# Sota0726/weather-Unet

Hardware: AMD Instinct MI355X
Metric: images/sec 256x256 cUNet fwd+bwd (higher is better)
Workload: dtype bf16; 1 GPU; cUNet 256x256 bf16 B=32/GPU, training step: fwd + bwd (dgrad+wgrad) + grad all-reduce + fused Adam; dropout p=0.3 on; random-init weights, 5-class one-hot, loss mean|G(x,c)-x|; global_batch=32, parallelism=dp1

## Files before the change

include/wu_kernels.h:

```cpp
#ifndef WU_KERNELS_H
#define WU_KERNELS_H

#include <stddef.h>
#include <stdint.h>

#ifdef __cplusplus
extern "C" {
#endif

#define WU_F32 0
#define WU_BF16 1

#define WU_ACT_NONE 0
#define WU_ACT_RELU 1
#define WU_ACT_LEAKY 2

const char* wu_last_error(void);
int wu_version(void);
int wu_cu_count(void);
int wu_set_option(int key, int value);
int wu_set_debug_buffer(void* p);
int wu_event_create(void** event_out);
int wu_event_destroy(void* event);
int wu_stream_order_after(void* waiter_stream, void* producer_stream, void* event);

int wu_stream_create_cu_mask(const unsigned* mask, int words, void** stream_out);
int wu_stream_destroy(void* stream);

int wu_pack_conv3x3(const float* w_oihw, void* w_fwd, void* w_dgrad, int Cout, int Cin,
                    const float* inv_sigma, int dtype, void* stream);
int wu_pack_conv3x3_multi(int n, const float* const* w_oihw, void* const* w_fwd, void* const* w_dgrad,
                          const int* Cout, const int* Cin, int dtype, void* stream);

size_t wu_spectral_norm_scratch_floats(int rows, int cols);
int wu_spectral_norm_fwd(const float* w, int rows, int cols, float* u, float* v, int power_iter, float eps,
                         float* sigma_out, float* w_eff, float* scratch, void* stream);
int wu_spectral_norm_bwd(const float* g, const float* w, const float* u, const float* v, const float* sigma,
                         float* dw, int rows, int cols, float* scratch, void* stream);
int wu_spectral_norm_fwd_multi(int n, const float* const* w, const int* rows, const int* cols, float* const* u, float* const* v,
                               int power_iter, float eps, float* const* sigma_out, float* const* w_eff, float* const* scratch,
                               float* const* u_save, float* const* v_save, void* stream);
int wu_spectral_norm_bwd_multi(int n, const float* const* g, const float* const* w, const float* const* u, const float* const* v,
                               const float* const* sigma, float* const* dw, const int* rows, const int* cols, float* const* scratch,
                               void* stream);

int wu_conv3x3_fwd(const void* x, int ldx, const void* w_packed, const float* bias, void* y, int ldy,
                   int N, int H, int W, int Cin, int Cout, int stride, int act,
                   const void* mask, int ldmask, int mask_act,
                   const void* egate, int ldegate, int egate_act, int dtype, void* stream);

int wu_conv3x3_gate_bits_supported(int H, int W, int ldx, int ldy, int Cin, int Cout, int dtype);
size_t wu_gate_bits_bytes(int N, int H, int W, int C);
int wu_conv3x3_fwd_bits(const void* x, int ldx, const void* w_packed, const float* bias, void* y, int ldy,
                        void* gate_bits_out, const void* egate_bits, int N, int H, int W, int Cin, int Cout,
                        int act, int dtype, void* stream);

int wu_conv3x3_relu_pool_fwd(const void* x, int ldx, const void* w_packed, const float* bias, void* y, int ldy,
                             void* pool, int ldpool, int N, int H, int W, int Cin, int Cout, int dtype, void* stream);
int wu_conv3x3_relu_pool_bits_fwd(const void* x, int ldx, const void* w_packed, const float* bias, void* y, int ldy,
                                  void* pool, int ldpool, void* gate_bits_out, void* sel_bits_out,
                                  int N, int H, int W, int Cin, int Cout, int dtype, void* stream);
int wu_conv3x3_small_supported(int N, int H, int W, int ldx, int ldy, int ldegate, int Cin, int Cout);
int wu_conv3x3_small_fwd(const void* x, int ldx, const void* w_chunked, const float* bias, void* y, int ldy,
                         const void* egate, int ldegate, int egate_act, int N, int H, int W, int Cin, int Cout, int act, void* stream);

int wu_conv3x3_relu_head_supported(int H, int W, int ldx, int ldy, int Cin, int Cout, int dtype);
int wu_conv3x3_relu_head_fwd(const void* x, int ldx, const void* w_packed, const float* bias, void* y, int ldy,
                             const float* head_w, const float* head_bias, float* out_nchw,
                             int N, int H, int W, int Cin, int Cout, int dtype, void* stream);
int wu_maxpool2_bwd_bits(const unsigned* gate_bits, const unsigned* sel_bits, const void* dy, int lddy, const void* dskip, int lddskip,
                         void* dx, int lddx, int N, int H, int W, int C, int dtype, void* stream);

size_t wu_conv3x3_wgrad_workspace(int N, int H, int W, int Cin, int Cout, int stride, int dtype);
int wu_conv3x3_wgrad(const void* x, int ldx, const void* dy, int lddy, const void* y, int ldy_, int act,
                     float* dw_oihw, float* dbias, void* workspace, size_t workspace_bytes,
                     int N, int H, int W, int Cin, int Cout, int stride, int accumulate,
                     int dtype, void* stream);

size_t wu_conv3x3_s2_dgrad_workspace(int N, int H, int W, int Cout, int dtype);
int wu_conv3x3_s2_dgrad(const void* dy, int lddy, const void* y, int ldy_, int act, const void* w_dgrad,
                        void* dx, int lddx, void* workspace, size_t workspace_bytes,
                        const void* egate, int ldegate, int egate_act,
                        int N, int H, int W, int Cin, int Cout, int dtype, void* stream);

int wu_act_gate(const void* g, int ldg, const void* y, int ldy, void* out, int ldo,
                int N, int H, int W, int C, int act, int dtype, void* stream);

int wu_conv3x3_c3_fwd(const float* x_nchw, const float* w_oihw, const float* bias, const float* inv_sigma,
                      void* y, int ldy, int out_nchw, int N, int H, int W, int Cout, int stride, int act,
                      int dtype, void* stream);
int wu_conv3x3_c3_gate_bits_supported(int N, int H, int W, int Cout, int stride, const float* bias, int dtype);
int wu_conv3x3_c3_fwd_bits(const float* x_nchw, const float* w_oihw, const float* bias, const float* inv_sigma,
                           void* y, int ldy, void* gate_bits_out, int N, int H, int W, int Cout, int stride, int dtype, void* stream);
int wu_conv3x3_c3_wgrad(const float* x_nchw, const void* dy, int lddy, int dy_nchw, const void* y, int ldy_,
                        int act, float* dw_oihw, float* dbias, void* workspace, size_t workspace_bytes,
                        int N, int H, int W, int Cout, int stride, int accumulate, int dtype, void* stream);
size_t wu_thin_workspace_bytes(void);
int wu_conv3x3_c3_dgrad(const void* dy, int lddy, int dy_nchw, const void* y, int ldy_, int act,
                        const float* w_oihw, const float* inv_sigma, float* dx_nchw, int N, int H, int W,
                        int Cout, int stride, int accumulate, int dtype, void* stream);

int wu_conv1x1_tanh_fwd(const void* x, int ldx, const float* w, const float* bias, float* out_nchw,
                        int N, int H, int W, int Cin, int dtype, void* stream);
int wu_conv1x1_tanh_bwd(const float* dout_nchw, const float* out_nchw, const void* x, int ldx, const float* w,
                        void* dx, int lddx, float* dw, float* dbias, void* workspace, size_t workspace_bytes,
                        int N, int H, int W, int Cin, int accumulate, int x_gate_act, int dtype, void* stream);

int wu_maxpool2_fwd(const void* x, int ldx, void* y, int ldy, int N, int H, int W, int C, int dtype, void* stream);
int wu_maxpool2_bwd(const void* x, int ldx, const void* dy, int lddy, const void* dskip, int lddskip,
                    void* dx, int lddx, int N, int H, int W, int C, int gate_act, int dtype, void* stream);

int wu_adain_style_fwd(const float* y, const float* w, const float* b, float eps, float* y_std, float* y_mean, float* y4,
                       int N, int C, int nc, void* stream);
int wu_adain_style_bwd(const float* d_std, const float* d_mean, const float* y, const float* y4, const float* y_std,
                       const float* y_mean, float* dw, float* db, int N, int C, int nc, int accumulate, void* stream);

int wu_adain_style_fwd_multi(int levels, const float* y, const float* const* w, const float* const* b, const float* eps,
                             float* const* y_std, float* const* y_mean, float* const* y4, int N, const int* C, int nc, void* stream);
int wu_adain_style_bwd_multi(int levels, const float* const* d_std, const float* const* d_mean, const float* y, const float* const* y4,
                             const float* const* y_std, const float* const* y_mean, float* const* dw, float* const* db,
                             int N, const int* C, int nc, int accumulate, void* stream);

#define WU_MAX_SPLITS 16
int wu_adain_stats(const void* x, int ldx, float* stats, float* scratch, int N, int H, int W, int C,
                   float eps, int dtype, void* stream);
int wu_adain_stats_as_batch(const void* x, int ldx, float* stats, float* scratch, int N, int H, int W, int C,
                            float eps, int split_batch, int dtype, void* stream);

int wu_adain_upcat_fwd(const void* x, int ldx, const float* stats, const float* y_std, const float* y_mean,
                       void* y, int ldy, int N, int H, int W, int C, float p_drop, uint64_t seed,
                       const uint64_t* seed_dev, uint8_t* mask_bits, int mask_is_input, int dtype, void* stream);
int wu_adain_upcat_sweep_fwd(const void* x, int ldx, int Bx, const float* stats, const float* y_std, const float* y_mean,
                             const void* skip, int ldskip, int Bs, int Cs, void* y, int ldy, int N, int H, int W, int C,
                             float p_drop, uint64_t seed, const uint64_t* seed_dev, int dtype, void* stream);
int wu_adain_upcat_bwd(const void* dy, int lddy, const void* x, int ldx, const float* stats, const float* y_std,
// ... 333 lines not shown
```

weather-unet_amd/csrc/conv3x3_mfma_v2.hip:

```cpp
#include <type_traits>

#include "wu_common.h"
#include "conv_internal.h"

#ifndef WU_CONV_STORE_AUX
#define WU_CONV_STORE_AUX 0
#endif

namespace {

struct K {
    static constexpr int TH = 16, TW = 32, P = TH * TW;
    static constexpr int HALO_W = TW + 2, HALO_H = TH + 2, HALO_PIX = HALO_W * HALO_H;
    static constexpr int H_PIECES = 40, H_BYTES = H_PIECES * 1024;
    static constexpr int W_REAL = 9 * 64 * 64 / 1024;
    static constexpr int W_PIECES = 40, W_BYTES = W_PIECES * 1024;
    static constexpr int BUF = H_BYTES + W_BYTES;
};
template <int NW_> struct KW {
    static constexpr int NW = NW_;
    static constexpr int RPW = K::TH / NW;
    static constexpr int NH = K::H_PIECES / NW;
    static constexpr int NWT = K::W_PIECES / NW;
    static constexpr int NP = NH + NWT;
    static constexpr int NST = K::P * 8 / (NW * 64);
};

struct V2Args {
    const bf16_t* x; const bf16_t* w; const float* bias; bf16_t* y; const bf16_t* egate;
    bf16_t* pool;
    unsigned* gbits;
    unsigned* sbits;
    const unsigned* egbits;
    int ldx, ldy, ldegate, egate_act, ldpool;
    int N, H, W, Cin, Cout, act;
    int tiles_x, tiles_y, cout_tiles, ntiles, prio_mode, strided;
    int w_resident;
    const float* head_w; const float* head_b; float* head_out;
    unsigned long long* dbg;
};

typedef float f32x2_t __attribute__((ext_vector_type(2)));
typedef short s16x2_t __attribute__((ext_vector_type(2)));
typedef unsigned short u16x2_t __attribute__((ext_vector_type(2)));
__device__ __forceinline__ uint32_t relu_bf16x2(uint32_t d) {
    const s16x2_t v = __builtin_elementwise_max(__builtin_bit_cast(s16x2_t, d), s16x2_t{0, 0});
    return __builtin_bit_cast(uint32_t, v);
}
__device__ __forceinline__ uint32_t relu_gate_bf16x2(uint32_t g, uint32_t y) {
    const u16x2_t nz = __builtin_elementwise_min(__builtin_bit_cast(u16x2_t, y), u16x2_t{1, 1});
    const u16x2_t m = u16x2_t{0, 0} - nz;
    const s16x2_t sg = __builtin_bit_cast(s16x2_t, y) >> s16x2_t{15, 15};
    return g & __builtin_bit_cast(uint32_t, m) & ~__builtin_bit_cast(uint32_t, sg);
}
__device__ __forceinline__ uint32_t max_u16x2(uint32_t a, uint32_t b) {
    const u16x2_t m = __builtin_elementwise_max(__builtin_bit_cast(u16x2_t, a), __builtin_bit_cast(u16x2_t, b));
    return __builtin_bit_cast(uint32_t, m);
}
__device__ __forceinline__ uint32_t nonzero_byte(const uint4& v) {
    uint32_t t0, t1, t2, t3;
    const uint32_t one = 0x00010001u;
    asm("v_pk_min_u16 %0, %1, %2" : "=&v"(t0) : "v"(v.x), "v"(one));
    asm("v_pk_min_u16 %0, %1, %2" : "=&v"(t1) : "v"(v.y), "v"(one));
    asm("v_pk_min_u16 %0, %1, %2" : "=&v"(t2) : "v"(v.z), "v"(one));
    asm("v_pk_min_u16 %0, %1, %2" : "=&v"(t3) : "v"(v.w), "v"(one));
    const uint32_t xx = ((t3 << 6) | t2 << 4) | ((t1 << 2) | t0);
    return (xx | (xx >> 15)) & 0xffu;
}
__device__ __forceinline__ uint32_t gate_mask2(int bits, int b) {
    const uint32_t lo = (uint32_t)((bits << (31 - b)) >> 31), hi = (uint32_t)((bits << (30 - b)) >> 31);
    return (lo & 0xffffu) | (hi << 16);
}
__device__ __forceinline__ float fast_tanh(float s) {
    const float e = __builtin_amdgcn_exp2f(s * 2.885390081777927f);
    return 1.f - 2.f * __builtin_amdgcn_rcpf(e + 1.f);
}
__device__ __forceinline__ void dma_wait_all() { asm volatile("s_waitcnt vmcnt(0)" ::: "memory"); }
__device__ __forceinline__ void mma(f32x16_t& acc, const uint4& a, const uint4& b) {
    acc = __builtin_amdgcn_mfma_f32_32x32x16_bf16(__builtin_bit_cast(bf16x8_t, a), __builtin_bit_cast(bf16x8_t, b), acc, 0, 0, 0);
}
__device__ __forceinline__ void mma16(f32x4_t& acc, const uint4& a, const uint4& b) {
    acc = __builtin_amdgcn_mfma_f32_16x16x32_bf16(__builtin_bit_cast(bf16x8_t, a), __builtin_bit_cast(bf16x8_t, b), acc, 0, 0, 0);
}
template <bool M16_, int RPW_> struct AccT { using type = f32x16_t[RPW_][2]; };
template <int RPW_> struct AccT<true, RPW_> { using type = f32x4_t[RPW_][2][4]; };

template <int NW, int GATED>
__global__ __launch_bounds__(NW * 64) void conv3x3_mfma_v2_kernel(const V2Args a) {
    using Q = KW<NW>;
// ... 272 lines not shown
                    load_step(1, af[1], bf[1]);
                    __builtin_amdgcn_sched_barrier(0);
                    mma_step(2);
                    __builtin_amdgcn_sched_barrier(0);
                }
#pragma unroll
                for (int step = 0; step < 18; ++step) {
                    if (step + 2 < 18) load_step(step + 2, af[(step + 2) % 3], bf[(step + 2) % 3]);
                    if (more && 2 * step < Q::NP) {
                        if (need_w || 2 * step < Q::NH) issue_piece(2 * step, c1, nxt);
                        if (2 * step + 1 < Q::NP && (need_w || 2 * step + 1 < Q::NH)) issue_piece(2 * step + 1, c1, nxt);
                    }
                    static_assert(2 * 5 >= Q::NP || NW != 8, "deferred stores must follow the last DMA piece");
                    if (FIRST && ov_pending && (GATED != 5 || has_y) && step >= 5 && step < 5 + Q::NST) store_ov(step - 5);
                    if (GATED == 3 && FIRST && ovb_pending && step >= 5 + Q::NST && step < 5 + Q::NST + Q::RPW) store_ovb(step - 5 - Q::NST);
                    if (GATED == 5 && FIRST && ovh_pending && step >= 5 + Q::NST && 2 * (step - 5 - Q::NST) < 3 * Q::RPW) {
                        store_ovh(2 * (step - 5 - Q::NST));
                        if (2 * (step - 5 - Q::NST) + 1 < 3 * Q::RPW) store_ovh(2 * (step - 5 - Q::NST) + 1);
                    }
                    __builtin_amdgcn_sched_barrier(0);
                    if (LAST || step < 18 - CARRY) mma_step(step % 3);
                    __builtin_amdgcn_sched_barrier(0);
                }
            } else {
                constexpr int NF = 12, NM = 32;
                auto load_frag = [&](int tap, int f, uint4 (&xf)[Q::RPW][2], uint4 (&wf)[4]) __attribute__((always_inline)) {
                    const int kh = tap / 3, kw = tap % 3;
                    if (f == 0 || f >= 9) {
                        const int cb = f == 0 ? 0 : f - 8;
                        wf[cb] = *(const uint4*)(lds + b16_lane + (tap * 64 + 16 * cb) * 64);
                    } else {
                        const int mi = (f - 1) >> 1, ph = (f - 1) & 1;
                        xf[mi][ph] = *(const uint4*)(lds + a16_lane[kw] + ((mi + kh) * K::HALO_W + 16 * ph) * 64);
                    }
                };
                auto mma_m = [&](int m, int slot) __attribute__((always_inline)) {
                    const int cb = m >> 3, mi = (m & 7) >> 1, ph = m & 1;
                    mma16(acc[mi][ph][cb], wr[slot][cb], xr[slot][mi][ph]);
                };
                const unsigned kill = more ? 0u : kWuOOB;
                if constexpr (FIRST) {
#pragma unroll
                    for (int f = 0; f < NF; ++f) load_frag(0, f, xr[0], wr[0]);
                } else {
#pragma unroll
                    for (int m = 0; m < NM; ++m) {
                        mma_m(m, 2);
                        if (m < NF) load_frag(0, m, xr[0], wr[0]);
                        __builtin_amdgcn_sched_barrier(0);
                    }
                }
#pragma unroll
                for (int tap = 0; tap < 9; ++tap) {
                    const int cur = tap % 3, nx = (tap + 1) % 3;
#pragma unroll
                    for (int m = 0; m < NM; ++m) {
                        if (LAST || tap < 9 - CARRY) mma_m(m, cur);
                        if (tap + 1 < 9 && m < NF) load_frag(tap + 1, m, xr[nx], wr[nx]);
                        if ((m == 15 || m == NM - 1) && 4 * tap < Q::NP) {
                            const int j0 = 4 * tap + (m == 15 ? 0 : 2);
                            if (j0 < Q::NP) issue_piece(j0, c1, nxt, kill);
                            if (j0 + 1 < Q::NP) issue_piece(j0 + 1, c1, nxt, kill);
                        }
                        static_assert(4 * 5 >= Q::NP || NW != 4, "deferred stores must follow the last DMA piece");
                        if (FIRST && (m == 15 || m == NM - 1) && ov_pending && tap >= 5) {
                            const int k0 = 4 * (tap - 5) + (m == 15 ? 0 : 2);
                            if (k0 + 1 < Q::NST) { store_ov(k0); store_ov(k0 + 1); }
                        }
                        if (GATED == 3 && FIRST && m == NM - 1 && ovb_pending && tap == 8) {
#pragma unroll
                            for (int mi = 0; mi < Q::RPW; ++mi) store_ovb(mi);
                        }
                        __builtin_amdgcn_sched_barrier(0);
                    }
                }
            }
            buf = nxt;
            if (FIRST && ov_pending) { stores_in_flight = ov_interior; bits_in_flight = ovb_pending; ov_pending = false; ovb_pending = false; ovh_pending = false; }
            if (FIRST) WU_STAMP(t_comp); else WU_STAMP(t_comp_rest);
        };
        do_chunk(0, std::true_type{}, std::false_type{});
        for (int c = 1; c + 1 < nchunks; ++c) do_chunk(c, std::false_type{}, std::false_type{});
        do_chunk(nchunks - 1, std::false_type{}, std::true_type{});
        if constexpr (M16) __syncthreads();

        const int n = cur.n;
        const int oh0 = cur.ty * K::TH, ow0 = cur.tx * K::TW, co0 = cur.ct * 64;
        WU_STAMP(t_epi_b1);
        const size_t img_pix = (size_t)n * a.H * a.W;
        auto epi_store = [&](auto act_tag, auto eg_tag, auto pool_tag) __attribute__((always_inline)) {
            constexpr int ACT = decltype(act_tag)::value, EG = decltype(eg_tag)::value;
            constexpr bool POOL = decltype(pool_tag)::value;
            constexpr int SCR_PITCH = 144;
            char* const scr = smem + (buf ^ 1) * K::BUF + wave * (Q::RPW * 32 * SCR_PITCH);
            if constexpr (M16) {
                static_assert(NW * Q::RPW * 32 * SCR_PITCH <= K::BUF, "transpose scratch must fit the free LDS buffer");
#pragma unroll
                for (int mi = 0; mi < Q::RPW; ++mi)
#pragma unroll
                    for (int ph = 0; ph < 2; ++ph)
#pragma unroll
                        for (int cb = 0; cb < 4; ++cb) {
                            const float4 bv = (GATED == 1 || GATED == 2) ? make_float4(0.f, 0.f, 0.f, 0.f) : b16[cb];
                            f32x2_t v0 = f32x2_t{acc[mi][ph][cb][0], acc[mi][ph][cb][1]} + f32x2_t{bv.x, bv.y};
                            f32x2_t v1 = f32x2_t{acc[mi][ph][cb][2], acc[mi][ph][cb][3]} + f32x2_t{bv.z, bv.w};
                            if (ACT == WU_ACT_LEAKY) {
                                const f32x2_t s0_ = v0 * 0.2f, s1_ = v1 * 0.2f;
                                v0 = f32x2_t{fmaxf(v0.x, s0_.x), fmaxf(v0.y, s0_.y)};
                                v1 = f32x2_t{fmaxf(v1.x, s1_.x), fmaxf(v1.y, s1_.y)};
                            }
                            uint2 o = make_uint2(pack_bf16x2(v0.x, v0.y), pack_bf16x2(v1.x, v1.y));
                            if (ACT == WU_ACT_RELU) { o.x = relu_bf16x2(o.x); o.y = relu_bf16x2(o.y); }
                            *(uint2*)(scr + (mi * 32 + 16 * ph + l15) * SCR_PITCH + (16 * cb + 4 * q16) * 2) = o;
                        }
            }
            unsigned gb[Q::RPW], sb[Q::RPW];
#pragma unroll
            for (int i = 0; i < Q::RPW; ++i) gb[i] = sb[i] = 0u;
            f32x16_t hacc[Q::RPW];
            if constexpr (GATED == 5) {
#pragma unroll
                for (int mi = 0; mi < Q::RPW; ++mi)
#pragma unroll
                    for (int i = 0; i < 16; ++i) hacc[mi][i] = 0.f;
            }
#pragma unroll
            for (int mp = 0; mp < Q::RPW / 2; ++mp) {
                const int ohe = oh0 + Q::RPW * wave + 2 * mp, ow = ow0 + l31;
#pragma unroll
                for (int ni = 0; ni < 2; ++ni)
#pragma unroll
                    for (int g = 0; g < 4; g += 2) {
                        uint4 vr[2];
#pragma unroll
                        for (int r = 0; r < 2; ++r) {
                            const int mi = 2 * mp + r;
                            uint4 v;
                            if constexpr (M16) {
                                v = *(const uint4*)(scr + (mi * 32 + l31) * SCR_PITCH + (32 * ni + 8 * g + 8 * lh) * 2);
                            } else {
                            uint32_t o[2][2];
#pragma unroll
                            for (int h = 0; h < 2; ++h) {
                                const float4 bv = (GATED == 1 || GATED == 2) ? make_float4(0.f, 0.f, 0.f, 0.f) : bvq[ni][g + h];
                                const int r0 = 4 * (g + h);
                                f32x2_t v0 = f32x2_t{acc[mi][ni][r0 + 0], acc[mi][ni][r0 + 1]} + f32x2_t{bv.x, bv.y};
                                f32x2_t v1 = f32x2_t{acc[mi][ni][r0 + 2], acc[mi][ni][r0 + 3]} + f32x2_t{bv.z, bv.w};
                                if (ACT == WU_ACT_LEAKY) {
                                    const f32x2_t s0_ = v0 * 0.2f, s1_ = v1 * 0.2f;
                                    v0 = f32x2_t{fmaxf(v0.x, s0_.x), fmaxf(v0.y, s0_.y)};
                                    v1 = f32x2_t{fmaxf(v1.x, s1_.x), fmaxf(v1.y, s1_.y)};
                                }
                                o[h][0] = pack_bf16x2(v0.x, v0.y);
                                o[h][1] = pack_bf16x2(v1.x, v1.y);
                                if (ACT == WU_ACT_RELU) { o[h][0] = relu_bf16x2(o[h][0]); o[h][1] = relu_bf16x2(o[h][1]); }
                            }
                            const auto s0 = __builtin_amdgcn_permlane32_swap(o[0][0], o[1][0], false, false);
                            const auto s1 = __builtin_amdgcn_permlane32_swap(o[0][1], o[1][1], false, false);
                            v = make_uint4(s0[0], s1[0], s0[1], s1[1]);
                            }
                            if (GATED == 2) {
                                const int by = (int)(egb[mi] >> (8 * (2 * ni + (g >> 1))));
                                v.x &= gate_mask2(by, 0);
                                v.y &= gate_mask2(by, 2);
                                v.z &= gate_mask2(by, 4);
                                v.w &= gate_mask2(by, 6);
                            } else if (EG != WU_ACT_NONE) {
                                const uint4 yv = egv[mi][ni][g >> 1];
                                if (EG == WU_ACT_RELU) {
                                    v.x = relu_gate_bf16x2(v.x, yv.x); v.y = relu_gate_bf16x2(v.y, yv.y);
                                    v.z = relu_gate_bf16x2(v.z, yv.z); v.w = relu_gate_bf16x2(v.w, yv.w);
                                } else {
                                    v = gate16<bf16_t>(v, yv, WU_ACT_LEAKY);
                                }
                            }
                            ov[((mp * 2 + ni) * 2 + (g >> 1)) * 2 + r] = v;
                            vr[r] = v;
                            if constexpr (GATED == 5) mma(hacc[mi], hA[2 * ni + (g >> 1)], v);
                            if ((GATED == 3 || GATED == 4) && ACT == WU_ACT_RELU)
                                gb[2 * mp + r] |= nonzero_byte(v) << (8 * (2 * ni + (g >> 1)));
                        }
                        if (POOL) {
                            uint4 m = make_uint4(max_u16x2(vr[0].x, vr[1].x), max_u16x2(vr[0].y, vr[1].y), max_u16x2(vr[0].z, vr[1].z), max_u16x2(vr[0].w, vr[1].w));
                            m.x = max_u16x2(m.x, (uint32_t)__builtin_amdgcn_mov_dpp((int)m.x, 0xB1, 0xF, 0xF, true));
                            m.y = max_u16x2(m.y, (uint32_t)__builtin_amdgcn_mov_dpp((int)m.y, 0xB1, 0xF, 0xF, true));
                            m.z = max_u16x2(m.z, (uint32_t)__builtin_amdgcn_mov_dpp((int)m.z, 0xB1, 0xF, 0xF, true));
                            m.w = max_u16x2(m.w, (uint32_t)__builtin_amdgcn_mov_dpp((int)m.w, 0xB1, 0xF, 0xF, true));
                            if ((l31 & 1) == 0 && ohe + 1 < a.H && ow + 1 < a.W) {
                                const int Hp = a.H >> 1, Wp = a.W >> 1;
                                *(uint4*)(a.pool + (((size_t)n * Hp + (ohe >> 1)) * Wp + (ow >> 1)) * a.ldpool + co0 + 8 * lh + 32 * ni + 8 * g) = m;
                            }
                            if constexpr (GATED == 4) {
                                const uint4 x0 = make_uint4(vr[0].x ^ m.x, vr[0].y ^ m.y, vr[0].z ^ m.z, vr[0].w ^ m.w);
                                const uint4 x1 = make_uint4(vr[1].x ^ m.x, vr[1].y ^ m.y, vr[1].z ^ m.z, vr[1].w ^ m.w);
                                const uint32_t eq0 = ~nonzero_byte(x0) & 0xffu, eq1 = ~nonzero_byte(x1) & 0xffu;
                                const uint32_t nb = (uint32_t)__builtin_amdgcn_mov_dpp((int)(eq0 | (eq1 << 8)), 0xB1, 0xF, 0xF, true);
                                const uint32_t oddm = (l31 & 1) ? 0xffu : 0u;
                                const uint32_t nb0 = nb & 0xffu, nb1 = (nb >> 8) & 0xffu;
                                const uint32_t s0 = eq0 & ~(nb0 & oddm);
                                const uint32_t s1 = eq1 & ~eq0 & ~nb0 & ~(nb1 & oddm);
                                sb[2 * mp] |= s0 << (8 * (2 * ni + (g >> 1)));
                                sb[2 * mp + 1] |= s1 << (8 * (2 * ni + (g >> 1)));
                            }
                        }
                    }
            }
            if constexpr (GATED == 4) {
#pragma unroll
                for (int mi = 0; mi < Q::RPW; ++mi) {
                    const int oh = oh0 + Q::RPW * wave + mi, ow = ow0 + l31;
                    if (oh < a.H && ow < a.W) {
                        const size_t wi = (((size_t)n * a.H + oh) * a.W + ow) * (2 * a.cout_tiles) + 2 * cur.ct + lh;
                        a.gbits[wi] = gb[mi];
                        a.sbits[wi] = sb[mi];
                    }
                }
            }
            if constexpr (GATED == 5) {
#pragma unroll
                for (int mi = 0; mi < Q::RPW; ++mi)
#pragma unroll
                    for (int c = 0; c < 3; ++c) ovh[mi][c] = fast_tanh((hacc[mi][c] + (hacc[mi][4 + c] + hacc[mi][8 + c])) + hbias[c]);
                ovh_off = (unsigned)(((size_t)n * 3 * a.H + oh0 + Q::RPW * wave) * a.W + ow0 + l31);
                ovh_pending = true;
            }
            if (GATED == 3 && ACT == WU_ACT_RELU) {
#pragma unroll
                for (int mi = 0; mi < Q::RPW; ++mi) ovb[mi] = gb[mi];
                ovb_off = (unsigned)((((size_t)n * a.H + oh0 + Q::RPW * wave) * a.W + ow0 + l31) * (2 * a.cout_tiles) + 2 * cur.ct + lh);
                ovb_pending = true;
            }
        };
        using A0 = std::integral_constant<int, WU_ACT_NONE>;
        using A1 = std::integral_constant<int, WU_ACT_RELU>;
        using A2 = std::integral_constant<int, WU_ACT_LEAKY>;
        using NoPool = std::false_type;
        if constexpr (GATED == 5) {
            epi_store(A1{}, A0{}, NoPool{});
        } else if constexpr (GATED == 4) {
            epi_store(A1{}, A0{}, std::true_type{});
        } else if constexpr (GATED == 3) {
            epi_store(A1{}, A0{}, NoPool{});
        } else if constexpr (GATED == 2) {
            epi_store(A0{}, A0{}, NoPool{});
        } else if constexpr (GATED == 1) {
            if (a.egate_act == WU_ACT_RELU) epi_store(A0{}, A1{}, NoPool{});
            else epi_store(A0{}, A2{}, NoPool{});
        } else {
            if (a.act == WU_ACT_RELU) {
                if (a.pool) epi_store(A1{}, A0{}, std::true_type{});
                else epi_store(A1{}, A0{}, NoPool{});
            }
            else if (a.act == WU_ACT_LEAKY) epi_store(A2{}, A0{}, NoPool{});
            else epi_store(A0{}, A0{}, NoPool{});
        }
        {
            const int ohw = oh0 + Q::RPW * wave, ow = ow0 + l31;
            ov_img = has_y ? a.y + img_pix * a.ldy : a.y;
            ov_off = (unsigned)(((ohw * a.W + ow) * a.ldy + co0 + 8 * lh) * 2);
            unsigned rows = 0;
#pragma unroll
            for (int rr = 0; rr < Q::RPW; ++rr) rows |= (ohw + rr < a.H && ow < a.W) ? (1u << rr) : 0u;
            ov_ok = 0;
#pragma unroll
            for (int k = 0; k < Q::NST; ++k) ov_ok |= ((rows >> (2 * (k >> 3) + (k & 1))) & 1u) << k;
            ov_interior = oh0 + K::TH <= a.H && ow0 + K::TW <= a.W;
            ov_pending = true;
        }
        WU_STAMP(t_epi_s);
        cur = advance(cur);
    }
    if (ov_pending) {
        if (GATED != 5 || has_y) {
#pragma unroll
            for (int k = 0; k < Q::NST; ++k) store_ov(k);
        }
        if (GATED == 5 && ovh_pending) {
#pragma unroll
            for (int k = 0; k < 3 * Q::RPW; ++k) store_ovh(k);
        }
        if (GATED == 3 && ovb_pending) {
#pragma unroll
            for (int mi = 0; mi < Q::RPW; ++mi) store_ovb(mi);
        }
    }
    if (NW == 4) dma_wait_all();
    if (a.dbg && lane == 0) {
        unsigned long long* d = a.dbg + ((size_t)blockIdx.x * 8 + wave) * 8;
        d[0] = t_wait; d[1] = t_comp + t_comp_rest; d[2] = __builtin_readcyclecounter() - t_k0; d[3] = __builtin_amdgcn_s_memrealtime() - t_r0;
         d[4] = t_epi_b2; d[5] = t_epi_s; d[6] = (unsigned long long)((t_end - t_begin + t_step - 1) / t_step); d[7] = nchunks | (t_comp << 8);
    }
#undef WU_STAMP
}

}

bool conv_v2_eligible(int H, int W, int ldx, int ldy, int Cin, int Cout, int stride, int dtype, bool masked) {
    return dtype == WU_BF16 && stride == 1 && !masked && W > 16 && W <= 4096 && Cin % 32 == 0 && Cin >= 64 && Cout % 64 == 0 &&
           (size_t)9 * Cout * Cin * 2 < (1ull << 31) && ((size_t)H * W + W + 2) * (size_t)ldx * 2 < (1ull << 31) &&
           ((size_t)H * W + W + 2) * (size_t)ldy * 2 < (1ull << 31);
}

int conv_v2_launch(const void* x, int ldx, const void* w, const float* bias, void* y, int ldy,
                   const void* egate, int ldegate, int egate_act, int N, int H, int W, int Cin, int Cout, int act, hipStream_t s,
                   void* pool, int ldpool, void* gate_bits_out, const void* egate_bits, void* sel_bits_out,
                   const float* head_w, const float* head_b, float* head_out) {
    V2Args a;
    a.head_w = head_w; a.head_b = head_b; a.head_out = head_out;
    a.pool = (bf16_t*)pool; a.ldpool = ldpool;
    a.x = (const bf16_t*)x; a.w = (const bf16_t*)w; a.bias = bias; a.y = (bf16_t*)y; a.egate = (const bf16_t*)egate;
    a.ldx = ldx; a.ldy = ldy; a.ldegate = ldegate; a.egate_act = egate_act; a.N = N; a.H = H; a.W = W; a.Cin = Cin; a.Cout = Cout; a.act = act;
    a.tiles_x = cdiv(W, K::TW); a.tiles_y = cdiv(H, K::TH); a.cout_tiles = Cout / 64;
    a.dbg = (unsigned long long*)g_wu_dbg_ptr;
    a.prio_mode = g_wu_opt[WU_OPT_CONV_PRIO];
    a.strided = g_wu_opt[WU_OPT_CONV_STRIDED];
    a.w_resident = 0;
    const long long ntiles = (long long)N * a.tiles_x * a.tiles_y * a.cout_tiles;
    if (ntiles >= (1ll << 31)) return -1;
    a.ntiles = (int)ntiles;
    const int cus = wu_num_cus();
    const long long grid = (ntiles < cus || !g_wu_opt[WU_OPT_CONV_PERSISTENT]) ? ntiles : cus;
    static thread_local bool attr_set = false;
    if (!attr_set) {
#define WU_V2_ATTR(NW_, G_) (void)hipFuncSetAttribute((const void*)conv3x3_mfma_v2_kernel<NW_, G_>, hipFuncAttributeMaxDynamicSharedMemorySize, 160 * 1024)
        WU_V2_ATTR(8, 5); WU_V2_ATTR(8, 0); WU_V2_ATTR(4, 0); WU_V2_ATTR(8, 1); WU_V2_ATTR(4, 1); WU_V2_ATTR(8, 2); WU_V2_ATTR(4, 2); WU_V2_ATTR(8, 3); WU_V2_ATTR(4, 3); WU_V2_ATTR(8, 4); WU_V2_ATTR(4, 4);
#undef WU_V2_ATTR
        attr_set = true;
    }
    const int mode = g_wu_opt[WU_OPT_CONV_V2];
    int gated = egate_bits ? 2 : ((egate != nullptr && egate_act != WU_ACT_NONE) ? 1 : 0);
    if (gated != 1) a.egate = nullptr;
    a.egbits = (const unsigned*)egate_bits;
    a.gbits = (gated == 0 && act == WU_ACT_RELU && !pool) ? (unsigned*)gate_bits_out : nullptr;
    a.sbits = nullptr;
    if (a.gbits) gated = 3;
    if (gated == 0 && act == WU_ACT_RELU && pool && gate_bits_out && sel_bits_out) {
        a.gbits = (unsigned*)gate_bits_out; a.sbits = (unsigned*)sel_bits_out;
        gated = 4;
    }
    if (head_out) {
        if (gated != 0 || act != WU_ACT_RELU || pool || Cout != 64 || Cin >= 256) return -2;
        gated = 5;
    }
    const bool nw4 = gated != 5 && (mode == 2 || (mode == 1 && Cin >= 256));
    a.w_resident = (!nw4 && Cin == 64 && a.cout_tiles == 1 && g_wu_opt[WU_OPT_CONV_W_RESIDENT]) ? 1 : 0;
#define WU_V2_GO(NW_, G_) hipLaunchKernelGGL((conv3x3_mfma_v2_kernel<NW_, G_>), dim3((int)grid), dim3(NW_ * 64), 2 * K::BUF, s, a)
    if (nw4) { if (gated == 4) WU_V2_GO(4, 4); else if (gated == 3) WU_V2_GO(4, 3); else if (gated == 2) WU_V2_GO(4, 2); else if (gated == 1) WU_V2_GO(4, 1); else WU_V2_GO(4, 0); }
    else { if (gated == 5) WU_V2_GO(8, 5); else if (gated == 4) WU_V2_GO(8, 4); else if (gated == 3) WU_V2_GO(8, 3); else if (gated == 2) WU_V2_GO(8, 2); else if (gated == 1) WU_V2_GO(8, 1); else WU_V2_GO(8, 0); }
#undef WU_V2_GO
    return 0;
}
```

weather-unet_amd/wu/_lib.py:

```python
import ctypes
import os

from ctypes import c_char_p, c_double, c_float, c_int, c_size_t, c_uint64, c_void_p, POINTER

_PKG = os.path.dirname(os.path.dirname(os.path.abspath(__file__)))
LIB_PATH = os.path.join(_PKG, "lib", "libwu_kernels.so")

F32, BF16 = 0, 1
ACT_NONE, ACT_RELU, ACT_LEAKY = 0, 1, 2
OPT_CONV_V2, OPT_CONV_PERSISTENT, OPT_WGRAD_V2 = 0, 1, 2
FAM_CONV_FWD, FAM_WGRAD, FAM_CONV_DGRAD, FAM_CONV_S2, FAM_WGRAD_S2, FAM_CONV1X1 = 1, 2, 3, 4, 5, 6
FAM_GRID = 7
FAMILY_KERNEL = {1: "conv3x3_mfma_v2_kernel (forward + data-gradient convs; generic conv3x3_mfma_kernel for fp32 / narrow images)",
                 2: "conv3x3_wgrad_v2_kernel (generic conv3x3_wgrad_kernel for fp32 / narrow images)",
                 3: "conv3x3_mfma_kernel<T,1,true> (in-kernel gated dgrad; unused by the fused graph)",
                 4: "stride-2 3x3 conv forward + data gradient: conv1x1_pw3_kernel<.., CONV> (gathered rows); conv3x3_mfma_kernel<T,2,false> / tap-list classes for 64-cout and fp32",
                 5: "conv3x3_wgrad_kernel<T,2>",
                 6: "pointwise convs (estimator): conv1x1_pw3_kernel; conv1x1_mfma_kernel<T> for strided / small / fp32"}

P, I, F, U64, SZ = c_void_p, c_int, c_float, c_uint64, c_size_t

SIGNATURES = {
    "wu_last_error": (c_char_p, []),
    "wu_version": (I, []),
    "wu_cu_count": (I, []),
    "wu_set_option": (I, [I, I]),
    "wu_set_debug_buffer": (I, [P]),
    "wu_stream_create_cu_mask": (I, [P, I, P]),
    "wu_stream_destroy": (I, [P]),
    "wu_spectral_norm_scratch_floats": (SZ, [I, I]),
    "wu_spectral_norm_fwd": (I, [P, I, I, P, P, I, F, P, P, P, P]),
    "wu_spectral_norm_bwd": (I, [P, P, P, P, P, P, I, I, P, P]),
    "wu_event_create": (I, [P]),
    "wu_event_destroy": (I, [P]),
    "wu_stream_order_after": (I, [P, P, P]),
    "wu_spectral_norm_fwd_multi": (I, [I, P, P, P, P, P, I, F, P, P, P, P, P, P]),
    "wu_spectral_norm_bwd_multi": (I, [I, P, P, P, P, P, P, P, P, P, P]),
    "wu_pack_conv3x3": (I, [P, P, P, I, I, P, I, P]),
    "wu_pack_conv3x3_multi": (I, [I, P, P, P, P, P, I, P]),
    "wu_conv3x3_fwd": (I, [P, I, P, P, P, I, I, I, I, I, I, I, I, P, I, I, P, I, I, I, P]),
    "wu_conv3x3_gate_bits_supported": (I, [I, I, I, I, I, I, I]),
    "wu_gate_bits_bytes": (SZ, [I, I, I, I]),
    "wu_conv3x3_fwd_bits": (I, [P, I, P, P, P, I, P, P, I, I, I, I, I, I, I, P]),
    "wu_conv3x3_relu_pool_fwd": (I, [P, I, P, P, P, I, P, I, I, I, I, I, I, I, P]),
    "wu_conv3x3_relu_pool_bits_fwd": (I, [P, I, P, P, P, I, P, I, P, P, I, I, I, I, I, I, P]),
    "wu_conv3x3_small_supported": (I, [I, I, I, I, I, I, I, I]),
    "wu_conv3x3_small_fwd": (I, [P, I, P, P, P, I, P, I, I, I, I, I, I, I, I, P]),
    "wu_conv3x3_relu_head_supported": (I, [I, I, I, I, I, I, I]),
    "wu_conv3x3_relu_head_fwd": (I, [P, I, P, P, P, I, P, P, P, I, I, I, I, I, I, P]),
    "wu_maxpool2_bwd_bits": (I, [P, P, P, I, P, I, P, I, I, I, I, I, I, P]),
    "wu_conv3x3_wgrad_workspace": (SZ, [I, I, I, I, I, I, I]),
    "wu_conv3x3_wgrad": (I, [P, I, P, I, P, I, I, P, P, P, SZ, I, I, I, I, I, I, I, I, P]),
    "wu_conv3x3_s2_dgrad_workspace": (SZ, [I, I, I, I, I]),
    "wu_conv3x3_s2_dgrad": (I, [P, I, P, I, I, P, P, I, P, SZ, P, I, I, I, I, I, I, I, I, P]),
    "wu_act_gate": (I, [P, I, P, I, P, I, I, I, I, I, I, I, P]),
    "wu_conv3x3_c3_fwd": (I, [P, P, P, P, P, I, I, I, I, I, I, I, I, I, P]),
    "wu_conv3x3_c3_gate_bits_supported": (I, [I, I, I, I, I, P, I]),
    "wu_conv3x3_c3_fwd_bits": (I, [P, P, P, P, P, I, P, I, I, I, I, I, I, P]),
    "wu_conv3x3_c3_wgrad": (I, [P, P, I, I, P, I, I, P, P, P, SZ, I, I, I, I, I, I, I, P]),
    "wu_thin_workspace_bytes": (SZ, []),
    "wu_conv3x3_c3_dgrad": (I, [P, I, I, P, I, I, P, P, P, I, I, I, I, I, I, I, P]),
    "wu_conv1x1_tanh_fwd": (I, [P, I, P, P, P, I, I, I, I, I, P]),
    "wu_conv1x1_tanh_bwd": (I, [P, P, P, I, P, P, I, P, P, P, SZ, I, I, I, I, I, I, I, P]),
    "wu_maxpool2_fwd": (I, [P, I, P, I, I, I, I, I, I, P]),
    "wu_maxpool2_bwd": (I, [P, I, P, I, P, I, P, I, I, I, I, I, I, I, P]),
    "wu_adain_style_fwd": (I, [P, P, P, F, P, P, P, I, I, I, P]),
    "wu_adain_style_bwd": (I, [P, P, P, P, P, P, P, P, I, I, I, I, P]),
    "wu_adain_style_fwd_multi": (I, [I, P, P, P, P, P, P, P, I, P, I, P]),
    "wu_adain_style_bwd_multi": (I, [I, P, P, P, P, P, P, P, P, I, P, I, I, P]),
    "wu_adain_stats": (I, [P, I, P, P, I, I, I, I, F, I, P]),
    "wu_adain_stats_as_batch": (I, [P, I, P, P, I, I, I, I, F, I, I, P]),
    "wu_adain_upcat_fwd": (I, [P, I, P, P, P, P, I, I, I, I, I, F, U64, P, P, I, I, P]),
    "wu_adain_upcat_sweep_fwd": (I, [P, I, I, P, P, P, P, I, I, I, P, I, I, I, I, I, F, U64, P, I, P]),
    "wu_adain_upcat_bwd": (I, [P, I, P, I, P, P, P, I, P, P, P, P, I, I, I, I, F, U64, P, I, I, P]),
    "wu_dropout_mask": (I, [P, I, I, I, I, F, U64, P]),
    "wu_l1_mean_scratch_floats": (SZ, []),
    "wu_l1_mean": (I, [P, P, P, P, P, ctypes.c_longlong, P]),
    "wu_sumpool_fwd": (I, [P, I, P, I, I, I, I, I, P]),
    "wu_sumpool_bwd": (I, [P, P, I, I, I, I, I, I, P]),
    "wu_nhwc_to_nchw_f32": (I, [P, I, P, I, I, I, I, I, P]),
    "wu_nchw_f32_to_nhwc": (I, [P, P, I, I, I, I, I, I, P]),
    "wu_conv1x1_fwd": (I, [P, I, P, P, P, I, P, I, I, I, I, I, I, I, I, I, I, I, I, I, P, I, I, I, P]),
    "wu_conv1x1_chain_supported": (I, [I, I, I, I]),
    "wu_conv1x1_chain": (I, [P, I, P, P, P, I, I, P, I, I, P, I, P, P, I, P, I, I, P, I, ctypes.c_longlong, I, I, I, I, P]),
    "wu_stem7x7_fwd": (I, [P, P, P, P, I, I, I, I, I, I, P]),
    "wu_stem7x7_dgrad": (I, [P, I, P, P, I, I, I, I, I, P]),
    "wu_maxpool3s2_fwd": (I, [P, I, P, I, P, I, I, I, I, I, P]),
    "wu_maxpool3s2_bwd": (I, [P, I, P, P, I, P, I, I, I, I, I, I, I, P]),
    "wu_bn_stats_workspace": (SZ, [ctypes.c_longlong, I, I]),
    "wu_bn_stats": (I, [P, I, ctypes.c_longlong, I, F, F, P, P, P, P, P, SZ, I, P]),
    "wu_bn_apply": (I, [P, I, P, P, P, P, I, P, P, P, P, I, P, I, ctypes.c_longlong, I, I, I, P]),
    "wu_bn_bwd_workspace": (SZ, [ctypes.c_longlong, I, I]),
    "wu_bn_bwd": (I, [P, I, P, I, I, P, I, P, P, P, P, P, I, P, I, P, P, P, P, P, I, P, I, ctypes.c_longlong, I, P, SZ, I, P]),
    "wu_conv1x1_wgrad_workspace": (SZ, [ctypes.c_longlong, I, I]),
    "wu_conv1x1_wgrad": (I, [P, I, P, I, P, P, SZ, I, I, I, I, I, I, I, I, I, I, P]),
    "wu_stem7x7_wgrad_workspace": (SZ, [I, I, I]),
    "wu_stem7x7_wgrad": (I, [P, P, I, P, P, SZ, I, I, I, I, I, P]),
    "wu_image_geo_bytes": (SZ, []),
    "wu_image_workspace_bytes": (SZ, [I, I, I]),
    "wu_image_geometry": (I, [P, P, P, SZ, P, P, I, I, I, I, P]),
    "wu_image_color_jitter": (I, [P, P, P, P, I, I, P]),
    "wu_jpeg_info_bytes": (SZ, []),
    "wu_jpeg_parse": (I, [P, SZ, P]),
    "wu_jpeg_entropy_decode": (I, [P, SZ, P, P, SZ, P]),
    "wu_jpeg_max_block_l1": (I, []),
    "wu_jpeg_desc_bytes": (SZ, []),
    "wu_jpeg_workspace_bytes": (SZ, [ctypes.c_longlong]),
    "wu_jpeg_reconstruct": (I, [P, P, P, P, P, SZ, P, I, I, I, I, P]),
    "wu_jpeg_scan_stage_bytes": (SZ, [P, SZ, I]),
    "wu_jpeg_scan_segments": (I, [P]),
    "wu_jpeg_scan_stage": (I, [P, SZ, P, I, P, SZ, P, SZ, P, P, P]),
    "wu_jpeg_huff_desc_bytes": (SZ, []),
    "wu_jpeg_huff_decode": (I, [P, P, P, P, P, P, P, I, I, P]),
    "wu_jpeg_enc_header_bytes": (SZ, []),
    "wu_jpeg_enc_header": (I, [I, I, I, I, P, SZ]),
    "wu_jpeg_enc_qtables": (I, [I, P]),
    "wu_jpeg_enc_desc_bytes": (SZ, []),
    "wu_jpeg_enc_workspace_bytes": (SZ, [I, I, I, I, ctypes.c_longlong]),
    "wu_jpeg_enc_out_stride": (SZ, [ctypes.c_longlong]),
    "wu_jpeg_enc_workspace_layout": (I, [I, I, I, I, ctypes.c_longlong, P]),
    "wu_jpeg_enc_encode": (I, [P, I, ctypes.c_longlong, ctypes.c_longlong, ctypes.c_longlong, ctypes.c_longlong, P, P, P, I, P, SZ, P, SZ, P, I, I, I, I, ctypes.c_longlong, P]),
    "wu_png_enc_desc_bytes": (SZ, []),
    "wu_png_enc_segment_bytes": (SZ, []),
    "wu_png_enc_workspace_bytes": (SZ, [I, I, I]),
    "wu_png_enc_out_stride": (SZ, [I, I]),
# ... 159 lines not shown
```

Baseline: 4133 images/sec.

## Replace LDS transpose in conv epilogue with permlane16 swaps; extend weight residency

The M16 epilogue of the v2 conv kernel no longer writes bias/activation results to an LDS scratch buffer and reads them back transposed behind a block-wide barrier. Instead each lane computes both phase halves in registers and exchanges them with permlane16_swap, which removes the __syncthreads and the LDS round trip. Launch planning moves into a shared conv_v2_plan helper that also allows weight-resident mode for multi-cout-tile persistent launches by trimming the grid to a multiple of cout tiles when the strided option is set. A plan query entry point and an A/B scratch benchmark script are added. Trimming the grid may leave some CUs idle, and the register-side transpose may raise register pressure.

```diff
diff --git a/include/wu_kernels.h b/include/wu_kernels.h
--- a/include/wu_kernels.h
+++ b/include/wu_kernels.h
@@ -51,6 +51,7 @@
 
 int wu_conv3x3_gate_bits_supported(int H, int W, int ldx, int ldy, int Cin, int Cout, int dtype);
 size_t wu_gate_bits_bytes(int N, int H, int W, int C);
+int wu_conv3x3_v2_plan(int N, int H, int W, int Cin, int Cout, int head, int* out);
 int wu_conv3x3_fwd_bits(const void* x, int ldx, const void* w_packed, const float* bias, void* y, int ldy,
                         void* gate_bits_out, const void* egate_bits, int N, int H, int W, int Cin, int Cout,
                         int act, int dtype, void* stream);
diff --git a/scratch/conv_v2_ab.py b/scratch/conv_v2_ab.py
--- /dev/null
+++ b/scratch/conv_v2_ab.py
@@ -0,0 +1,177 @@
+import json
+import os
+import statistics
+import sys
+
+LAYERS = [("down1.2", 64, 64, 1, "pool"), ("down2.0", 64, 128, 2, "bits"), ("down2.2", 128, 128, 2, "pool"), ("down3.0", 128, 256, 4, "bits"),
+          ("down3.2", 256, 256, 4, "pool"), ("down4.0", 256, 512, 8, "bits"), ("down4.2", 512, 512, 8, "plain"), ("up3.0", 768, 256, 4, "bits"),
+          ("up3.2", 256, 256, 4, "plain"), ("up2.0", 384, 128, 2, "bits"), ("up2.2", 128, 128, 2, "plain"), ("up1.0", 192, 64, 1, "bits"),
+          ("up1.2", 64, 64, 1, "head")]
+OPT_CONV_V2, OPT_W_RESIDENT = 0, 11
+
+
+def _setup():
+    root = os.path.join(os.path.dirname(os.path.abspath(__file__)), "..")
+    sys.path.insert(0, os.path.join(root, "weather-unet_amd"))
+    import torch
+    from wu import _lib, kernels as K
+    from wu.layout import empty_nhwc
+    _lib.load()
+    return torch, _lib, K, empty_nhwc
+
+
+def _launches(torch, K, empty_nhwc, name, ci, co, s, kind, B):
+    dev, bf = torch.device("cuda:0"), torch.bfloat16
+
+    def act(c, relu):
+        t = torch.relu(torch.randn((B, s, s, c), device=dev)) if relu else torch.rand((B, s, s, c), device=dev) * 2 - 1
+        return t.to(bf).permute(0, 3, 1, 2)
+
+    x, gy = act(ci, kind != "bits" or name.startswith("down")), act(co, False)
+    w = (torch.rand((co, ci, 3, 3), device=dev) * 2 - 1) * 0.05
+    wf, wd = K.pack_conv3x3(w, 1)
+    bias = torch.zeros(co, device=dev)
+    y, dx = empty_nhwc(B, co, s, s, bf, dev), empty_nhwc(B, ci, s, s, bf, dev)
+    if kind == "pool":
+        pl = empty_nhwc(B, co, s // 2, s // 2, bf, dev)
+        gbp, sbp = K.gate_bits_alloc(y), K.gate_bits_alloc(y)
+        fwd = lambda: K.conv3x3_relu_pool_bits(x, wf, bias, y, pl, gbp, sbp)
+    elif kind == "bits":
+        gbo = K.gate_bits_alloc(y)
+        fwd = lambda: K.conv3x3_bits(x, wf, bias, y, 1, gate_bits_out=gbo)
+    elif kind == "head":
+        hw3, hb3 = torch.rand((3, 64), device=dev) - 0.5, torch.zeros(3, device=dev)
+        himg = torch.empty((B, 3, s, s), device=dev)
+        fwd = lambda: K.conv3x3_relu_head(x, wf, bias, y, hw3, hb3, himg)
+    else:
+        fwd = lambda: K.conv3x3(x, wf, bias, y, 1, 1)
+    if kind == "bits":
+        dgrad = lambda: K.conv3x3(gy, wd, None, dx)
+    else:
+        gbi = torch.randint(-2**31, 2**31 - 1, (K.gate_bits_alloc(dx).numel(),), dtype=torch.int32, device=dev)
+        dgrad = lambda: K.conv3x3_bits(gy, wd, None, dx, egate_bits=gbi)
+    return fwd, dgrad
+
+
+def _warm(torch, K, empty_nhwc, B):
+    dev = torch.device("cuda:0")
+    wx = (torch.rand((B, 128, 128, 128), device=dev) * 2 - 1).to(torch.bfloat16).permute(0, 3, 1, 2)
+    wy = empty_nhwc(B, 128, 128, 128, torch.bfloat16, dev)
+    wf, _ = K.pack_conv3x3((torch.rand((128, 128, 3, 3), device=dev) * 2 - 1) * 0.05, 1)
+    for _ in range(1500):
+        K.conv3x3(wx, wf, None, wy, 1, 1)
+    torch.cuda.synchronize()
+
+
+def table(out, reps):
+    torch, _lib, K, empty_nhwc = _setup()
+    B, S = 32, 256
+    _warm(torch, K, empty_nhwc, B)
+
+    def run(fn, inner=4):
+        for _ in range(2):
+            fn()
+        torch.cuda.synchronize()
+        ts = []
+        for _ in range(reps):
+            e0, e1 = torch.cuda.Event(enable_timing=True), torch.cuda.Event(enable_timing=True)
+            e0.record()
+            for _ in range(inner):
+                fn()
+            e1.record()
+            torch.cuda.synchronize()
+            ts.append(round(e0.elapsed_time(e1) * 1e3 / inner, 2))
+        return ts
+
+    rows = []
+    for rep in range(2):
+        rows.clear()
+        for name, ci, co, div, kind in LAYERS:
+            fwd, dgrad = _launches(torch, K, empty_nhwc, name, ci, co, S // div, kind, B)
+            rows.append((f"{name} fwd {ci}->{co} @{S // div}", 4 if ci >= 256 else 8, run(fwd)))
+            rows.append((f"{name} dgrad {co}->{ci} @{S // div}", 4 if co >= 256 else 8, run(dgrad)))
+            extra = []
+            if name == "up1.0":
+                extra = [(f"{name} fwd {ci}->{co} @{S // div} [option 0 = 2: 4 waves]", OPT_CONV_V2, 2, 1, fwd, 4),
+                         (f"{name} dgrad {co}->{ci} @{S // div} [option 11 = 0: weights not resident]", OPT_W_RESIDENT, 0, 1, dgrad, 8)]
+            if name == "down2.0":
+                extra = [(f"{name} fwd {ci}->{co} @{S // div} [option 11 = 0: weights not resident]", OPT_W_RESIDENT, 0, 1, fwd, 8)]
+            for label, key, val, dflt, fn, waves in extra:
+                _lib.call("wu_set_option", key, val)
+                try:
+                    rows.append((label, waves, run(fn)))
+                finally:
+                    _lib.call("wu_set_option", key, dflt)
+            del fwd, dgrad
+    with open(out, "a") as fh:
+        for label, waves, ts in rows:
+            fh.write(json.dumps({"kind": "launch", "lib": _lib.LOADED_PATH, "launch": label, "waves": waves, "us": ts}) + "\n")
+    print(f"{_lib.LOADED_PATH}: {len(rows)} launches x {reps} samples -> {out}")
+
+
+def stamps(out):
+    torch, _lib, K, empty_nhwc = _setup()
+    B, S = 32, 256
+    dev = torch.device("cuda:0")
+    _warm(torch, K, empty_nhwc, B)
+    dbg = torch.zeros(256 * 8 * 8, dtype=torch.int64, device=dev)
+    with open(out, "a") as fh:
+        for want, which in (("down3.2", 0), ("up1.0", 1)):
+            name, ci, co, div, kind = next(l for l in LAYERS if l[0] == want)
+            fn = _launches(torch, K, empty_nhwc, name, ci, co, S // div, kind, B)[which]
+            waves = 4 if (ci if which == 0 else co) >= 256 else 8
+            for _ in range(3):
+                fn()
+            torch.cuda.synchronize()
+            dbg.zero_()
+            _lib.call("wu_set_debug_buffer", dbg.data_ptr())
+            try:
+                fn()
+                torch.cuda.synchronize()
+            finally:
+                _lib.call("wu_set_debug_buffer", None)
+            d = dbg.view(256, 8, 8)[:, :waves].cpu()
+            live = d[:, 0, 6] > 0
+            d = d[live]
+            tiles = d[:, :, 6].double()
+            chunks = int(d[0, 0, 7].item()) & 255
+            first = (d[:, :, 7] >> 8).double()
+            per_tile = lambda v: round((v.double() / tiles).mean().item())
+            rec = {"kind": "stamps", "lib": _lib.LOADED_PATH, "launch": f"{name} {'fwd' if which == 0 else 'dgrad'}", "waves": waves, "workgroups": int(live.sum()),
+                   "tiles_per_workgroup": [int(tiles.min().item()), int(tiles.max().item())], "chunks_per_tile": chunks,
+                   "clock_ghz": round((d[:, 0, 2].double() / d[:, 0, 3].double()).median().item() * 0.1, 3),
+                   "cycles_per_tile": {"total": per_tile(d[:, :, 2]), "dma_wait": per_tile(d[:, :, 0]), "chunk_top_barrier": per_tile(d[:, :, 4]),
+                                       "compute": per_tile(d[:, :, 1]), "compute_first_chunk": round((first / tiles).mean().item()),
+                                       "epilogue": per_tile(d[:, :, 5]),
+                                       "unstamped": per_tile(d[:, :, 2] - d[:, :, 0] - d[:, :, 1] - d[:, :, 4] - d[:, :, 5])}}
+            fh.write(json.dumps(rec) + "\n")
+            print(json.dumps(rec))
+
+
+def summary(files):
+    recs = [json.loads(l) for f in files for l in open(f) if l.strip()]
+    side = lambda r: "old" if "_oldlib" in r["lib"] else ("var" if "_varlib" in r["lib"] else "new")
+    launches = {}
+    for r in recs:
+        if r["kind"] == "launch":
+            launches.setdefault(r["launch"], {}).setdefault(side(r), []).extend(r["us"])
+    print("| launch | waves | old median | old min | new median | new min | samples | new median < old min |\n|---|---|---|---|---|---|---|---|")
+    waves = {r["launch"]: r["waves"] for r in recs if r["kind"] == "launch"}
+    for k, v in launches.items():
+        o, n = v.get("old", []), v.get("new", [])
+        f = lambda xs, fn: f"{fn(xs):.1f}" if xs else "-"
+        verdict = ("yes" if statistics.median(n) < min(o) else "no") if o and n else "-"
+        print(f"| {k} | {waves[k]} | {f(o, statistics.median)} | {f(o, min)} | {f(n, statistics.median)} | {f(n, min)} | {len(o)} / {len(n)} | {verdict} |")
+    for r in recs:
+        if r["kind"] == "stamps":
+            print(side(r), json.dumps({k: v for k, v in r.items() if k not in ("kind", "lib")}))
+
+
+if __name__ == "__main__":
+    mode = sys.argv[1]
+    if mode == "table":
+        table(sys.argv[2], int(sys.argv[3]) if len(sys.argv) > 3 else 7)
+    elif mode == "stamps":
+        stamps(sys.argv[2])
+    else:
+        summary(sys.argv[2:])
diff --git a/weather-unet_amd/csrc/conv3x3_mfma_v2.hip b/weather-unet_amd/csrc/conv3x3_mfma_v2.hip
--- a/weather-unet_amd/csrc/conv3x3_mfma_v2.hip
+++ b/weather-unet_amd/csrc/conv3x3_mfma_v2.hip
@@ -5,6 +5,9 @@
 
 #ifndef WU_CONV_STORE_AUX
 #define WU_CONV_STORE_AUX 0
+#endif
+#ifndef WU_CONV_V2_NW4_CIN
+#define WU_CONV_V2_NW4_CIN 256
 #endif
 
 namespace {
@@ -443,8 +446,6 @@
         do_chunk(0, std::true_type{}, std::false_type{});
         for (int c = 1; c + 1 < nchunks; ++c) do_chunk(c, std::false_type{}, std::false_type{});
         do_chunk(nchunks - 1, std::false_type{}, std::true_type{});
-        if constexpr (M16) __syncthreads();
-
         const int n = cur.n;
         const int oh0 = cur.ty * K::TH, ow0 = cur.tx * K::TW, co0 = cur.ct * 64;
         WU_STAMP(t_epi_b1);
@@ -452,29 +453,6 @@
         auto epi_store = [&](auto act_tag, auto eg_tag, auto pool_tag) __attribute__((always_inline)) {
             constexpr int ACT = decltype(act_tag)::value, EG = decltype(eg_tag)::value;
             constexpr bool POOL = decltype(pool_tag)::value;
-            constexpr int SCR_PITCH = 144;
-            char* const scr = smem + (buf ^ 1) * K::BUF + wave * (Q::RPW * 32 * SCR_PITCH);
-            if constexpr (M16) {
-                static_assert(NW * Q::RPW * 32 * SCR_PITCH <= K::BUF, "transpose scratch must fit the free LDS buffer");
-#pragma unroll
-                for (int mi = 0; mi < Q::RPW; ++mi)
-#pragma unroll
-                    for (int ph = 0; ph < 2; ++ph)
-#pragma unroll
-                        for (int cb = 0; cb < 4; ++cb) {
-                            const float4 bv = (GATED == 1 || GATED == 2) ? make_float4(0.f, 0.f, 0.f, 0.f) : b16[cb];
-                            f32x2_t v0 = f32x2_t{acc[mi][ph][cb][0], acc[mi][ph][cb][1]} + f32x2_t{bv.x, bv.y};
-                            f32x2_t v1 = f32x2_t{acc[mi][ph][cb][2], acc[mi][ph][cb][3]} + f32x2_t{bv.z, bv.w};
-                            if (ACT == WU_ACT_LEAKY) {
-                                const f32x2_t s0_ = v0 * 0.2f, s1_ = v1 * 0.2f;
-                                v0 = f32x2_t{fmaxf(v0.x, s0_.x), fmaxf(v0.y, s0_.y)};
-                                v1 = f32x2_t{fmaxf(v1.x, s1_.x), fmaxf(v1.y, s1_.y)};
-                            }
-                            uint2 o = make_uint2(pack_bf16x2(v0.x, v0.y), pack_bf16x2(v1.x, v1.y));
-                            if (ACT == WU_ACT_RELU) { o.x = relu_bf16x2(o.x); o.y = relu_bf16x2(o.y); }
-                            *(uint2*)(scr + (mi * 32 + 16 * ph + l15) * SCR_PITCH + (16 * cb + 4 * q16) * 2) = o;
-                        }
-            }
             unsigned gb[Q::RPW], sb[Q::RPW];
 #pragma unroll
             for (int i = 0; i < Q::RPW; ++i) gb[i] = sb[i] = 0u;
@@ -498,7 +476,25 @@
                             const int mi = 2 * mp + r;
                             uint4 v;
                             if constexpr (M16) {
-                                v = *(const uint4*)(scr + (mi * 32 + l31) * SCR_PITCH + (32 * ni + 8 * g + 8 * lh) * 2);
+                                const int cb = 2 * ni + (g >> 1);
+                                uint32_t o[2][2];
+#pragma unroll
+                                for (int ph = 0; ph < 2; ++ph) {
+                                    const float4 bv = (GATED == 1 || GATED == 2) ? make_float4(0.f, 0.f, 0.f, 0.f) : b16[cb];
+                                    f32x2_t v0 = f32x2_t{acc[mi][ph][cb][0], acc[mi][ph][cb][1]} + f32x2_t{bv.x, bv.y};
+                                    f32x2_t v1 = f32x2_t{acc[mi][ph][cb][2], acc[mi][ph][cb][3]} + f32x2_t{bv.z, bv.w};
+                                    if (ACT == WU_ACT_LEAKY) {
+                                        const f32x2_t s0_ = v0 * 0.2f, s1_ = v1 * 0.2f;
+                                        v0 = f32x2_t{fmaxf(v0.x, s0_.x), fmaxf(v0.y, s0_.y)};
+                                        v1 = f32x2_t{fmaxf(v1.x, s1_.x), fmaxf(v1.y, s1_.y)};
+                                    }
+                                    o[ph][0] = pack_bf16x2(v0.x, v0.y);
+                                    o[ph][1] = pack_bf16x2(v1.x, v1.y);
+                                    if (ACT == WU_ACT_RELU) { o[ph][0] = relu_bf16x2(o[ph][0]); o[ph][1] = relu_bf16x2(o[ph][1]); }
+                                }
+                                const auto s0 = __builtin_amdgcn_permlane16_swap(o[0][0], o[1][0], false, false);
+                                const auto s1 = __builtin_amdgcn_permlane16_swap(o[0][1], o[1][1], false, false);
+                                v = make_uint4(s0[0], s1[0], s0[1], s1[1]);
                             } else {
                             uint32_t o[2][2];
 #pragma unroll
@@ -662,6 +658,32 @@
            ((size_t)H * W + W + 2) * (size_t)ldy * 2 < (1ull << 31);
 }
 
+namespace {
+struct V2Plan { int waves, grid, w_resident; };
+V2Plan conv_v2_plan(int N, int H, int W, int Cin, int Cout, bool head) {
+    const int cout_tiles = Cout / 64;
+    const long long ntiles = (long long)N * cdiv(W, K::TW) * cdiv(H, K::TH) * cout_tiles;
+    const int cus = wu_num_cus();
+    const bool walk = ntiles >= cus && g_wu_opt[WU_OPT_CONV_PERSISTENT];
+    long long grid = walk ? cus : ntiles;
+    const int mode = g_wu_opt[WU_OPT_CONV_V2];
+    const bool nw4 = !head && (mode == 2 || (mode == 1 && Cin >= WU_CONV_V2_NW4_CIN));
+    int res = 0;
+    if (!nw4 && Cin == 64 && g_wu_opt[WU_OPT_CONV_W_RESIDENT]) {
+        if (cout_tiles == 1 || !walk) res = 1;
+        else if (g_wu_opt[WU_OPT_CONV_STRIDED] && grid >= cout_tiles) { grid -= grid % cout_tiles; res = 1; }
+    }
+    return V2Plan{nw4 ? 4 : 8, (int)(grid < (1ll << 31) ? grid : 0), res};
+}
+}
+
+extern "C" int wu_conv3x3_v2_plan(int N, int H, int W, int Cin, int Cout, int head, int* out) {
+    WU_REQUIRE(out && N > 0 && H > 0 && W > 0 && Cin >= 64 && Cout >= 64 && Cout % 64 == 0, "conv3x3_v2_plan: bad args");
+    const V2Plan p = conv_v2_plan(N, H, W, Cin, Cout, head != 0);
+    out[0] = p.waves; out[1] = p.grid; out[2] = p.w_resident; out[3] = Cout / 64;
+    return 0;
+}
+
 int conv_v2_launch(const void* x, int ldx, const void* w, const float* bias, void* y, int ldy,
                    const void* egate, int ldegate, int egate_act, int N, int H, int W, int Cin, int Cout, int act, hipStream_t s,
                    void* pool, int ldpool, void* gate_bits_out, const void* egate_bits, void* sel_bits_out,
@@ -679,8 +701,6 @@
     const long long ntiles = (long long)N * a.tiles_x * a.tiles_y * a.cout_tiles;
     if (ntiles >= (1ll << 31)) return -1;
     a.ntiles = (int)ntiles;
-    const int cus = wu_num_cus();
-    const long long grid = (ntiles < cus || !g_wu_opt[WU_OPT_CONV_PERSISTENT]) ? ntiles : cus;
     static thread_local bool attr_set = false;
     if (!attr_set) {
 #define WU_V2_ATTR(NW_, G_) (void)hipFuncSetAttribute((const void*)conv3x3_mfma_v2_kernel<NW_, G_>, hipFuncAttributeMaxDynamicSharedMemorySize, 160 * 1024)
@@ -688,7 +708,6 @@
 #undef WU_V2_ATTR
         attr_set = true;
     }
-    const int mode = g_wu_opt[WU_OPT_CONV_V2];
     int gated = egate_bits ? 2 : ((egate != nullptr && egate_act != WU_ACT_NONE) ? 1 : 0);
     if (gated != 1) a.egate = nullptr;
     a.egbits = (const unsigned*)egate_bits;
@@ -703,9 +722,11 @@
         if (gated != 0 || act != WU_ACT_RELU || pool || Cout != 64 || Cin >= 256) return -2;
         gated = 5;
     }
-    const bool nw4 = gated != 5 && (mode == 2 || (mode == 1 && Cin >= 256));
-    a.w_resident = (!nw4 && Cin == 64 && a.cout_tiles == 1 && g_wu_opt[WU_OPT_CONV_W_RESIDENT]) ? 1 : 0;
-#define WU_V2_GO(NW_, G_) hipLaunchKernelGGL((conv3x3_mfma_v2_kernel<NW_, G_>), dim3((int)grid), dim3(NW_ * 64), 2 * K::BUF, s, a)
+    const V2Plan plan = conv_v2_plan(N, H, W, Cin, Cout, gated == 5);
+    const bool nw4 = plan.waves == 4;
+    const int grid = plan.grid;
+    a.w_resident = plan.w_resident;
+#define WU_V2_GO(NW_, G_) hipLaunchKernelGGL((conv3x3_mfma_v2_kernel<NW_, G_>), dim3(grid), dim3(NW_ * 64), 2 * K::BUF, s, a)
     if (nw4) { if (gated == 4) WU_V2_GO(4, 4); else if (gated == 3) WU_V2_GO(4, 3); else if (gated == 2) WU_V2_GO(4, 2); else if (gated == 1) WU_V2_GO(4, 1); else WU_V2_GO(4, 0); }
     else { if (gated == 5) WU_V2_GO(8, 5); else if (gated == 4) WU_V2_GO(8, 4); else if (gated == 3) WU_V2_GO(8, 3); else if (gated == 2) WU_V2_GO(8, 2); else if (gated == 1) WU_V2_GO(8, 1); else WU_V2_GO(8, 0); }
 #undef WU_V2_GO
diff --git a/weather-unet_amd/wu/_lib.py b/weather-unet_amd/wu/_lib.py
--- a/weather-unet_amd/wu/_lib.py
+++ b/weather-unet_amd/wu/_lib.py
@@ -41,6 +41,7 @@
     "wu_conv3x3_fwd": (I, [P, I, P, P, P, I, I, I, I, I, I, I, I, P, I, I, P, I, I, I, P]),
     "wu_conv3x3_gate_bits_supported": (I, [I, I, I, I, I, I, I]),
     "wu_gate_bits_bytes": (SZ, [I, I, I, I]),
+    "wu_conv3x3_v2_plan": (I, [I, I, I, I, I, I, P]),
     "wu_conv3x3_fwd_bits": (I, [P, I, P, P, P, I, P, P, I, I, I, I, I, I, I, P]),
     "wu_conv3x3_relu_pool_fwd": (I, [P, I, P, P, P, I, P, I, I, I, I, I, I, I, P]),
     "wu_conv3x3_relu_pool_bits_fwd": (I, [P, I, P, P, P, I, P, I, P, P, I, I, I, I, I, I, P]),
```

Result: faster. 4195 images/sec, median of 6 (+1.5%).
